# mobvoi/lstm_ctc

Measured on AMD Instinct MI355X. Metric: acoustic frames/sec (whole node), 5xBiLSTM-1024 CTC, higher is better.
Workload: dtype f32

## Files before the change

lstm_ctc_amd/csrc/lstm.hip:

```cpp
#include "common.h"
#include <stdlib.h>
#include <string.h>
#include <mutex>
#include <type_traits>

typedef float f32x4 __attribute__((ext_vector_type(4)));

static unsigned long long *g_lstm_dbg = nullptr;
typedef int x_i32x4 __attribute__((ext_vector_type(4)));
__device__ f32x4 x_buffer_load_b128(x_i32x4 rsrc, int voffset, int soffset, int aux) __asm("llvm.amdgcn.raw.buffer.load.v4f32");
__device__ void x_buffer_store_b128(f32x4 v, x_i32x4 rsrc, int voffset, int soffset, int aux) __asm("llvm.amdgcn.raw.buffer.store.v4f32");
typedef float x_f32x2v __attribute__((ext_vector_type(2)));
__device__ x_f32x2v x_buffer_load_b64(x_i32x4 rsrc, int voffset, int soffset, int aux) __asm("llvm.amdgcn.raw.buffer.load.v2f32");
__device__ float x_buffer_load_b32(x_i32x4 rsrc, int voffset, int soffset, int aux) __asm("llvm.amdgcn.raw.buffer.load.f32");
__device__ void x_buffer_store_b32(float v, x_i32x4 rsrc, int voffset, int soffset, int aux) __asm("llvm.amdgcn.raw.buffer.store.f32");
__device__ void x_buffer_store_b64(x_f32x2v v, x_i32x4 rsrc, int voffset, int soffset, int aux) __asm("llvm.amdgcn.raw.buffer.store.v2f32");
__device__ void x_buffer_store_b16(short v, x_i32x4 rsrc, int voffset, int soffset, int aux) __asm("llvm.amdgcn.raw.buffer.store.i16");

namespace {

constexpr int NTHREADS = 256;
constexpr int NWAVES = 4;

struct DirFwd {
// ... 1562 lines not shown
    for (int kb = 0; kb < NKB; ++kb) {
        const int k0 = uh * HALF + wave * (16 * NKB) + kb * 16 + 4 * lk;
#pragma unroll
        for (int c = 0; c < 8; ++c) {
            const int unit = ((c & 1) ? (1 - uh) : uh) * HALF + slot * 16 + li;
            const float *src = d.R + (size_t)k0 * G + (unit >> 3) * 32 + (c >> 1) * 8 + (unit & 7);
            wreg[kb][c].x = src[0]; wreg[kb][c].y = src[(size_t)G];
            wreg[kb][c].z = src[(size_t)2 * G]; wreg[kb][c].w = src[(size_t)3 * G];
        }
    }
    float *hxme = p.hx + (size_t)xcc * 2 * 2 * X_HXBUF;
    const x_i32x4 px_rs = x_rsrc(p.px, (unsigned)(X_PX_FLOATS * sizeof(float)));
    const int pxcell = ((slot * 16 + i) * 16 + ul) * 32;
    const x_i32x4 hx_rs = x_rsrc(hxme, (unsigned)(2 * 2 * X_HXBUF * sizeof(float)));
    const int hx_vo = (lk * 16 + li) * 16;
    const int hx_so = __builtin_amdgcn_readfirstlane(wave * NKB * 1024);
    const int hx_pub = (ul & 3) == 0 ? ((slot * 4 + (ul >> 2)) * 16 + i) * 16 : 0x7ffffff0;
    constexpr int X_NT = 2;
    auto publish_state = [&](int sg, int s, float h) {
        const int v = (int)((__float_as_uint(h) & ~1u) | p_gen_bit((unsigned)s + 1u));
        const f32x4 g = {__int_as_float(__builtin_amdgcn_mov_dpp(v, 0x00, 0xf, 0xf, true)),
                         __int_as_float(__builtin_amdgcn_mov_dpp(v, 0x55, 0xf, 0xf, true)),
                         __int_as_float(__builtin_amdgcn_mov_dpp(v, 0xaa, 0xf, 0xf, true)),
                         __int_as_float(__builtin_amdgcn_mov_dpp(v, 0xff, 0xf, 0xf, true))};
        x_buffer_store_b128(g, hx_rs, hx_pub, (sg * 2 + (s & 1)) * (X_HXBUF * 4), 0);
    };
    XGroup grp[2];
    grp[0].cprev = grp[1].cprev = 0.f;
    f32x4 a[NKB];
    bool failed = false;
    int step = 0;

    const x_i32x4 zx_rs = x_rsrc(d.zx, (unsigned)((size_t)T * B * G * sizeof(float)));
    const x_i32x4 cs_rs = x_rsrc(d.cs, (unsigned)((size_t)T * B * N * sizeof(float)));
    const x_i32x4 hs_rs = x_rsrc(d.hs, (unsigned)((size_t)T * B * N * sizeof(float)));
    int zvo[2], svo[2];
#pragma unroll
    for (int sg = 0; sg < 2; ++sg) { zvo[sg] = (brow[sg] * G + (int)zcol) * 4; svo[sg] = (brow[sg] * N + n) * 4; }
    auto load_zx = [&](int sg, int s) {
        const int zo = (int)((unsigned)(d.reverse ? (T - 1 - s) : s) * (unsigned)(B * G * 4));
#pragma unroll
        for (int g = 0; g < 4; ++g) grp[sg].z[g] = x_buffer_load_b32(zx_rs, zvo[sg] + 32 * g, zo, 0);
    };
    auto gates = [&](int sg, int s, const float (&zsum)[4]) {
        const int t = d.reverse ? (T - 1 - s) : s;
        const float cp = grp[sg].cprev;
        const float ia = lc_sigmoid(__builtin_fmaf(wi, cp, grp[sg].z[0] + zsum[0]));
        const float fa = lc_sigmoid(__builtin_fmaf(wf, cp, (grp[sg].z[2] + zsum[2]) + p.forget_bias));
        const float ja = lc_tanh(grp[sg].z[1] + zsum[1]);
        const float cn = __builtin_fmaf(fa, cp, ia * ja);
        const float oa = lc_sigmoid(__builtin_fmaf(wo, cn, grp[sg].z[3] + zsum[3]));
        const bool act = t < len[sg];
        const float h = act ? oa * lc_tanh(cn) : 0.f;
        grp[sg].cprev = act ? cn : 0.f;
        publish_state(sg, s, h);
        if (valid[sg]) {
            float *zrow = d.zx + ((size_t)t * B + brow[sg]) * G + zcol;
            const size_t so = ((size_t)t * B + brow[sg]) * N + n;
            zrow[0] = act ? ia : 0.f; zrow[8] = act ? ja : 0.f; zrow[16] = act ? fa : 0.f; zrow[24] = act ? oa : 0.f;
            d.cs[so] = grp[sg].cprev;
            d.hs[so] = h;
        }
    };
    auto request_state = [&](int sg, int s) {
        const int so = hx_so + (sg * 2 + ((s + 1) & 1)) * (X_HXBUF * 4);
#pragma unroll
        for (int kb = 0; kb < NKB; ++kb) a[kb] = x_buffer_load_b128(hx_rs, hx_vo, so + kb * 1024, X_NT);
    };
    auto state_stale = [&](int s, const f32x4 (&av)[NKB]) {
        unsigned stale = 0;
#pragma unroll
        for (int kb = 0; kb < NKB; ++kb) stale |= __float_as_uint(av[kb].x) ^ p_gen_bit((unsigned)s);
        return __builtin_amdgcn_ballot_w64((stale & 1u) != 0) != 0;
    };

    load_zx(0, 0);
    load_zx(1, 0);
    {
        const float zero[4] = {0.f, 0.f, 0.f, 0.f};
        gates(0, 0, zero);
        gates(1, 0, zero);
    }
    if (T > 1) { load_zx(0, 1); load_zx(1, 1); }
    __syncthreads();
    auto half = [&](auto XC, auto PC, int s) -> bool {
        constexpr int X = decltype(XC)::value, Y = X ^ 1;
        constexpr bool POST = decltype(PC)::value;
        const int k = 2 * s + X, sy = (k - 1) >> 1;
        step = s;
        float *partX = p_lds + (size_t)X * (NWAVES * 16 * X_LDP), *partY = p_lds + (size_t)Y * (NWAVES * 16 * X_LDP);
        if (X == 0) LC_XSTAMP(0); else LC_XSTAMP(8);
        {
            if (k == 2) request_state(X, s);
            if (state_stale(s, a)) {
                unsigned nspin = 0;
                for (;;) {
                    if (!p_keep_waiting(nspin, p.spin_limit, p.ctl)) { failed = true; break; }
                    asm volatile("" ::: "memory");
                    request_state(X, s);
                    if (!state_stale(s, a)) break;
                }
            }
        }
        if (X == 0) LC_XSTAMP(1); else LC_XSTAMP(9);
        f32x4 acc[8];
#pragma unroll
        for (int c = 0; c < 8; ++c) acc[c] = (f32x4){0.f, 0.f, 0.f, 0.f};
        asm volatile("s_nop 7" : "+v"(acc[0]), "+v"(acc[1]), "+v"(acc[2]), "+v"(acc[3]), "+v"(acc[4]), "+v"(acc[5]),
                                 "+v"(acc[6]), "+v"(acc[7]) : : "memory");
        float pl[4][NWAVES], pr[4][NWAVES], zrem[4], zsum[4] = {0.f, 0.f, 0.f, 0.f};
        f32x4 rv0 = {0.f, 0.f, 0.f, 0.f}, rv1 = rv0;
        float gx = 0.f, ge = 0.f, ia = 0.f, fa = 0.f, ja = 0.f, cn = 0.f, oa = 0.f, th = 0.f, hh = 0.f;
        bool act = false;
        const float tag_y = __uint_as_float((unsigned)sy);
        const int pxblk = (sy + 1) & 1;
        const int pxsend = (((xcc ^ 1) * 2 + Y) * 2 + pxblk) * X_PXBLK + pxcell, pxrecv = ((xcc * 2 + Y) * 2 + pxblk) * X_PXBLK + pxcell;
        const int ty = d.reverse ? (T - 1 - sy) : sy;
        const unsigned tyu = (unsigned)sy;
        auto late = [&]() {
            return __builtin_amdgcn_ballot_w64(((__float_as_uint(rv0.y) ^ tyu) | (__float_as_uint(rv0.w) ^ tyu) |
                                                (__float_as_uint(rv1.y) ^ tyu) | (__float_as_uint(rv1.w) ^ tyu)) != 0) != 0;
        };
        constexpr int C_RECV = NKB - 4 > 2 ? NKB - 4 : 2, C_SUM = C_RECV + 1, C_GATE = C_RECV + 2;
        static_assert(C_GATE < NKB, "five chunks at least");
        auto mic = [&](auto KC, int m) {
            constexpr int KB = decltype(KC)::value;
            XGroup &q = grp[Y];
            if constexpr (KB == 0 && POST) {
                const int g = m >> 3, w = (m >> 1) & 3;
                if (m & 1) pr[g][w] = partY[(size_t)(w * 16 + i) * X_LDP + g * 32 + 16 + ul];
                else pl[g][w] = partY[(size_t)(w * 16 + i) * X_LDP + g * 32 + ul];
            } else if constexpr (KB == 1 && POST) {
                if (m < 8) {
                    const int g = m >> 1;
                    if (m & 1) zrem[g] = (pr[g][0] + pr[g][1]) + (pr[g][2] + pr[g][3]);
                    else q.zloc[g] = (pl[g][0] + pl[g][1]) + (pl[g][2] + pl[g][3]);
                } else if (m == 8) {
                    x_buffer_store_b128((f32x4){zrem[0], tag_y, zrem[1], tag_y}, px_rs, pxsend, 0, X_SYS);
                } else if (m == 9) {
                    x_buffer_store_b128((f32x4){zrem[2], tag_y, zrem[3], tag_y}, px_rs, pxsend + 16, 0, X_SYS);
                }
            } else if constexpr (KB == C_RECV && POST) {
                if (m == 0) rv0 = x_buffer_load_b128(px_rs, pxrecv, 0, X_SYS);
                else if (m == 1) rv1 = x_buffer_load_b128(px_rs, pxrecv + 16, 0, X_SYS);
            } else if constexpr (KB == C_SUM && POST) {
                if (m == 0) {
                    if (late()) {
                        unsigned nspin = 0;
                        for (;;) {
                            if (!p_keep_waiting(nspin, p.spin_limit, p.ctl)) { failed = true; break; }
                            rv0 = x_buffer_load_b128(px_rs, pxrecv, 0, X_SYS);
                            rv1 = x_buffer_load_b128(px_rs, pxrecv + 16, 0, X_SYS);
                            if (!late()) break;
                        }
                    }
                } else if (m == 1) {
                    zsum[0] = q.zloc[0] + rv0.x; zsum[1] = q.zloc[1] + rv0.z;
                    zsum[2] = q.zloc[2] + rv1.x; zsum[3] = q.zloc[3] + rv1.z;
                }
            } else if constexpr (KB == C_GATE && POST) {
                const float cp = q.cprev;
                if (m == 0) gx = __builtin_fmaf(wi, cp, q.z[0] + zsum[0]);
                else if (m == 1) ge = __builtin_amdgcn_exp2f(-1.44269504088896341f * gx);
                else if (m == 2) ia = __builtin_amdgcn_rcpf(1.0f + ge);
                else if (m == 3) gx = __builtin_fmaf(wf, cp, (q.z[2] + zsum[2]) + p.forget_bias);
                else if (m == 4) ge = __builtin_amdgcn_exp2f(-1.44269504088896341f * gx);
                else if (m == 5) fa = __builtin_amdgcn_rcpf(1.0f + ge);
                else if (m == 6) { gx = q.z[1] + zsum[1]; ge = __builtin_amdgcn_exp2f(-2.88539008177792681f * fabsf(gx)); }
                else if (m == 7) ja = copysignf((1.0f - ge) * __builtin_amdgcn_rcpf(1.0f + ge), gx);
                else if (m == 8) { cn = __builtin_fmaf(fa, cp, ia * ja); gx = __builtin_fmaf(wo, cn, q.z[3] + zsum[3]); }
                else if (m == 9) ge = __builtin_amdgcn_exp2f(-1.44269504088896341f * gx);
                else if (m == 10) oa = __builtin_amdgcn_rcpf(1.0f + ge);
                else if (m == 11) ge = __builtin_amdgcn_exp2f(-2.88539008177792681f * fabsf(cn));
                else if (m == 12) th = copysignf((1.0f - ge) * __builtin_amdgcn_rcpf(1.0f + ge), cn);
                else if (m == 13) { act = ty < len[Y]; hh = act ? oa * th : 0.f; q.cprev = act ? cn : 0.f; }
                else if (m == 14) {
                    publish_state(Y, sy, hh);
                } else if (m == 16 || m == 18 || m == 20) {
                    if (valid[Y]) {
                        const int zo = (int)((unsigned)ty * (unsigned)(B * G * 4)), so = ty * B * N * 4;
                        if (m == 16) {
                            x_buffer_store_b32(act ? ia : 0.f, zx_rs, zvo[Y], zo, 0);
                            x_buffer_store_b32(act ? ja : 0.f, zx_rs, zvo[Y] + 32, zo, 0);
                        } else if (m == 18) {
                            x_buffer_store_b32(act ? fa : 0.f, zx_rs, zvo[Y] + 64, zo, 0);
                            x_buffer_store_b32(act ? oa : 0.f, zx_rs, zvo[Y] + 96, zo, 0);
                        } else {
                            x_buffer_store_b32(q.cprev, cs_rs, svo[Y], so, 0);
                            x_buffer_store_b32(hh, hs_rs, svo[Y], so, 0);
                        }
                    }
                } else if (m == 22) {
                    if (sy + 1 < T) load_zx(Y, sy + 1);
                }
            } else if constexpr (KB == C_GATE && !POST) {
                if (m == 0 && sy + 1 < T) load_zx(Y, sy + 1);
            }
        };
#define LC_XMFMA(ACC, A, W) asm volatile("v_mfma_f32_16x16x4_f32 %0, %1, %2, %0" : "+v"(ACC) : "v"(A), "a"(W))
#define LC_XCHUNK(KB)                                                                                              \
    _Pragma("unroll") for (int c = 0; c < 8; ++c) {                                                                \
        LC_XMFMA(acc[c], a[KB].x, wreg[KB][c].x); mic(std::integral_constant<int, KB>(), c);                       \
        __builtin_amdgcn_sched_barrier(0);                                                                         \
    }                                                                                                              \
    _Pragma("unroll") for (int c = 0; c < 8; ++c) {                                                                \
        LC_XMFMA(acc[c], a[KB].y, wreg[KB][c].y); mic(std::integral_constant<int, KB>(), 8 + c);                   \
        __builtin_amdgcn_sched_barrier(0);                                                                         \
    }                                                                                                              \
    _Pragma("unroll") for (int c = 0; c < 8; ++c) {                                                                \
        LC_XMFMA(acc[c], a[KB].z, wreg[KB][c].z); mic(std::integral_constant<int, KB>(), 16 + c);                  \
        __builtin_amdgcn_sched_barrier(0);                                                                         \
    }                                                                                                              \
    _Pragma("unroll") for (int c = 0; c < 8; ++c) {                                                                \
        LC_XMFMA(acc[c], a[KB].w, wreg[KB][c].w); mic(std::integral_constant<int, KB>(), 24 + c);                  \
        __builtin_amdgcn_sched_barrier(0);                                                                         \
    }
        LC_XCHUNK(0) LC_XCHUNK(1) LC_XCHUNK(2) LC_XCHUNK(3) LC_XCHUNK(4)
        if constexpr (NKB > 5) { LC_XCHUNK(5) }
        if constexpr (NKB > 6) { LC_XCHUNK(6) }
        if constexpr (NKB > 7) { LC_XCHUNK(7) }
#undef LC_XCHUNK
#undef LC_XMFMA
        asm volatile("s_nop 15\n\ts_nop 15\n\ts_nop 7" : "+v"(acc[0]), "+v"(acc[1]), "+v"(acc[2]), "+v"(acc[3]), "+v"(acc[4]),
                                                         "+v"(acc[5]), "+v"(acc[6]), "+v"(acc[7]) : : "memory");
        if (X == 0) LC_XSTAMP(2); else LC_XSTAMP(10);
#pragma unroll
        for (int c = 0; c < 8; ++c)
#pragma unroll
            for (int r = 0; r < 4; ++r) partX[(size_t)(wave * 16 + lk * 4 + r) * X_LDP + c * 16 + li] = acc[c][r];
        if (k + 1 < 2 * T) request_state(Y, (k + 1) >> 1);
        if (failed) s_fail = 1;
        __syncthreads();
        if (X == 0) LC_XSTAMP(3); else LC_XSTAMP(11);
        return s_fail == 0;
    };
    {
        const std::integral_constant<int, 0> g0;
        const std::integral_constant<int, 1> g1;
        const std::true_type post;
        bool ok = T > 1 && half(g0, std::false_type(), 1) && half(g1, post, 1);
        for (int s = 2; ok && s < T; ++s) ok = half(g0, post, s) && half(g1, post, s);
    }
    if (T > 1 && !s_fail) {
        const int Y = 1, sy = T - 1;
        const float *partY = p_lds + (size_t)Y * (NWAVES * 16 * X_LDP);
        const float tag_y = __uint_as_float((unsigned)sy);
        const int pxblk = (sy + 1) & 1;
        const int pxsend = (((xcc ^ 1) * 2 + Y) * 2 + pxblk) * X_PXBLK + pxcell, pxrecv = ((xcc * 2 + Y) * 2 + pxblk) * X_PXBLK + pxcell;
        float zrem[4], zsum[4];
#pragma unroll
        for (int g = 0; g < 4; ++g) {
            const float *q = partY + (size_t)i * X_LDP + g * 32 + ul;
            grp[Y].zloc[g] = (q[0] + q[(size_t)16 * X_LDP]) + (q[(size_t)32 * X_LDP] + q[(size_t)48 * X_LDP]);
            zrem[g] = (q[16] + q[(size_t)16 * X_LDP + 16]) + (q[(size_t)32 * X_LDP + 16] + q[(size_t)48 * X_LDP + 16]);
        }
        x_buffer_store_b128((f32x4){zrem[0], tag_y, zrem[1], tag_y}, px_rs, pxsend, 0, X_SYS);
        x_buffer_store_b128((f32x4){zrem[2], tag_y, zrem[3], tag_y}, px_rs, pxsend + 16, 0, X_SYS);
        unsigned nspin = 0;
        const unsigned ty = (unsigned)sy;
        f32x4 rv0, rv1;
        for (;;) {
            rv0 = x_buffer_load_b128(px_rs, pxrecv, 0, X_SYS);
            rv1 = x_buffer_load_b128(px_rs, pxrecv + 16, 0, X_SYS);
            if (__builtin_amdgcn_ballot_w64(((__float_as_uint(rv0.y) ^ ty) | (__float_as_uint(rv0.w) ^ ty) |
                                             (__float_as_uint(rv1.y) ^ ty) | (__float_as_uint(rv1.w) ^ ty)) != 0) == 0) break;
            if (!p_keep_waiting(nspin, p.spin_limit, p.ctl)) { failed = true; break; }
        }
        zsum[0] = grp[Y].zloc[0] + rv0.x; zsum[1] = grp[Y].zloc[1] + rv0.z;
        zsum[2] = grp[Y].zloc[2] + rv1.x; zsum[3] = grp[Y].zloc[3] + rv1.z;
        gates(Y, sy, zsum);
        if (__syncthreads_or(failed ? 1 : 0)) s_fail = 1;
    }
    if (s_fail && threadIdx.x == 0) p_report_failure(p.ctl);
}

constexpr int XB_LDP = 36;
typedef float x_f32x2 __attribute__((ext_vector_type(2)));
struct XBwdArgs {
    DirBwd d[2];
    const int *seq_len;
    int row_base[2];
    int T, B;
    unsigned spin_limit;
    PCtl *ctl;
    float *dzx;
    float *px;
    float *upg[2];
    unsigned long long *dbg;
};
constexpr int XB_DZBUF = 512 * 16 * 4;
constexpr size_t XB_DZX_FLOATS = (size_t)8 * 2 * 2 * XB_DZBUF;
constexpr int XB_PXBLK = 32 * 16 * 16 * 8;
constexpr size_t XB_PX_FLOATS = (size_t)8 * 2 * 2 * XB_PXBLK / 4;

struct XBGroup {
    float ia, ja, fa, oa, dh, cn, cp;
    float dc;
    float dloc;
};
template <int NKB>
__global__ __launch_bounds__(P_THREADS) void lstm_bwd_pair_kernel(XBwdArgs p)
{
    extern __shared__ __attribute__((aligned(16))) float p_lds[];
    __shared__ int s_slot, s_fail;
    const int xcc = p_xcc_id();
    if (xcc >= 8) return;
    if (threadIdx.x == 0) {
        s_fail = 0;
        s_slot = (int)__hip_atomic_fetch_add(&p.ctl->claim[xcc], 1u, __ATOMIC_RELAXED, __HIP_MEMORY_SCOPE_AGENT);
    }
    __syncthreads();
    const int slot = s_slot;
    constexpr int HALF = 64 * NKB, NSLOT = 4 * NKB, NB = 4 * NKB;
    if (slot >= NSLOT) return;
    const int dirx = xcc >> 2, rh = (xcc >> 1) & 1, uh = xcc & 1;
    const DirBwd &d = p.d[dirx];
    constexpr int N = 128 * NKB, G = 4 * N;
    const int B = p.B, T = p.T;
    const int lane = threadIdx.x & 63, wave = __builtin_amdgcn_readfirstlane(threadIdx.x >> 6);
    const int li = lane & 15, lk = lane >> 4;
    const int i = threadIdx.x >> 4, ul = threadIdx.x & 15;
    const int n = uh * HALF + slot * 16 + ul;
    const float wi = d.w_i ? d.w_i[n] : 0.f, wf = d.w_f ? d.w_f[n] : 0.f, wo = d.w_o ? d.w_o[n] : 0.f;
    const int cbase = (n >> 3) * 32 + (n & 7);
    int brow[2], len[2];
    bool valid[2];
#pragma unroll
    for (int sg = 0; sg < 2; ++sg) {
        const int b = p.row_base[dirx] + rh * 32 + sg * 16 + i;
        valid[sg] = b < B;
        brow[sg] = min(b, B - 1);
        len[sg] = valid[sg] ? p.seq_len[brow[sg]] : 0;
    }
    struct XW { float x, y, z, w; };
    XW wreg[NB][2];
#pragma unroll
    for (int kb = 0; kb < NB; ++kb) {
        const int ku = uh * HALF + wave * (16 * NKB) + kb * 4 + lk;
        const float *src0 = d.RT + (size_t)((ku >> 3) * 32 + (ku & 7)) * N;
#pragma unroll
        for (int c = 0; c < 2; ++c) {
            const int ou = (c ? (1 - uh) : uh) * HALF + slot * 16 + li;
            wreg[kb][c].x = src0[ou]; wreg[kb][c].y = src0[(size_t)8 * N + ou];
            wreg[kb][c].z = src0[(size_t)16 * N + ou]; wreg[kb][c].w = src0[(size_t)24 * N + ou];
        }
    }
    float *dzme = p.dzx + (size_t)xcc * 2 * 2 * XB_DZBUF;
    const x_i32x4 px_rs = x_rsrc(p.px, (unsigned)(XB_PX_FLOATS * sizeof(float)));
    const int pxcell = ((slot * 16 + i) * 16 + ul) * 8;
    const x_i32x4 dz_rs = x_rsrc(dzme, (unsigned)(2 * 2 * XB_DZBUF * sizeof(float)));
    const int dz_vo = (lk * 16 + li) * 16;
    const int dz_so = __builtin_amdgcn_readfirstlane(wave * NKB * 4096);
    const int dz_pub = ((slot * 16 + ul) * 16 + i) * 16;
    constexpr int X_NT = 2;
    XBGroup grp[2];
    grp[0].dc = grp[1].dc = 0.f;
    f32x4 a[2][16];
    float ug[2][7] = {{0.f, 0.f, 0.f, 0.f, 0.f, 0.f, 0.f}, {0.f, 0.f, 0.f, 0.f, 0.f, 0.f, 0.f}};
    auto uacc = [&](int sg, float gi, float gj, float gf, float go, float cp, float cn) {
        ug[sg][0] = __builtin_fmaf(gi, cp, ug[sg][0]); ug[sg][1] = __builtin_fmaf(gf, cp, ug[sg][1]);
        ug[sg][2] = __builtin_fmaf(go, cn, ug[sg][2]);
        ug[sg][3] += gi; ug[sg][4] += gj; ug[sg][5] += gf; ug[sg][6] += go;
    };
    bool failed = false;
    int step = 0;

    auto tof = [&](int s) { return d.reverse ? s : (T - 1 - s); };
    const x_i32x4 g_rs = x_rsrc(d.gates, (unsigned)((size_t)T * B * G * sizeof(float)));
    const x_i32x4 dh_rs = x_rsrc(d.dh, (unsigned)((size_t)T * B * N * sizeof(float)));
    const x_i32x4 cs_rs = x_rsrc(d.cs, (unsigned)((size_t)T * B * N * sizeof(float)));
    int gvo[2], svo[2];
#pragma unroll
    for (int sg = 0; sg < 2; ++sg) { gvo[sg] = (brow[sg] * G + cbase) * 4; svo[sg] = (brow[sg] * N + n) * 4; }
    auto load_gates = [&](int sg, int s) {
        const int go = (int)((unsigned)tof(s) * (unsigned)(B * G * 4));
        grp[sg].ia = x_buffer_load_b32(g_rs, gvo[sg], go, 0); grp[sg].ja = x_buffer_load_b32(g_rs, gvo[sg] + 32, go, 0);
        grp[sg].fa = x_buffer_load_b32(g_rs, gvo[sg] + 64, go, 0); grp[sg].oa = x_buffer_load_b32(g_rs, gvo[sg] + 96, go, 0);
    };
    auto load_rest = [&](int sg, int s) {
        const int t = tof(s);
        const int tprev = d.reverse ? t + 1 : t - 1;
        const bool has_prev = d.reverse ? (t + 1 < T) : (t > 0);
        grp[sg].dh = x_buffer_load_b32(dh_rs, svo[sg], t * B * N * 4, 0);
        grp[sg].cn = x_buffer_load_b32(cs_rs, svo[sg], t * B * N * 4, 0);
        const float cpv = x_buffer_load_b32(cs_rs, svo[sg], (has_prev ? tprev : t) * B * N * 4, 0);
        grp[sg].cp = has_prev ? cpv : 0.f;
    };
    auto load_operands = [&](int sg, int s) { load_gates(sg, s); load_rest(sg, s); };
    auto derivs = [&](int sg, int s, float drec) {
        const int t = tof(s);
        const XBGroup &q = grp[sg];
        const float dh = q.dh + drec;
        const float tc = lc_tanh(q.cn);
        const float do_pre = dh * tc * q.oa * (1.f - q.oa);
        const float dcn = __builtin_fmaf(do_pre, wo, __builtin_fmaf(dh * q.oa, __builtin_fmaf(-tc, tc, 1.f), q.dc));
        const float di_pre = dcn * q.ja * q.ia * (1.f - q.ia);
        const float dj_pre = dcn * q.ia * __builtin_fmaf(-q.ja, q.ja, 1.f);
        const float df_pre = dcn * q.cp * q.fa * (1.f - q.fa);
        const bool act = t < len[sg];
        const float odi = act ? di_pre : 0.f, odj = act ? dj_pre : 0.f, odf = act ? df_pre : 0.f, odo = act ? do_pre : 0.f;
        uacc(sg, odi, odj, odf, odo, q.cp, q.cn);
        grp[sg].dc = act ? __builtin_fmaf(df_pre, wf, __builtin_fmaf(di_pre, wi, dcn * q.fa)) : q.dc;
        x_buffer_store_b128(p_with_lsb_tag(odi, odj, odf, odo, p_gen_bit((unsigned)s + 1u)), dz_rs, dz_pub,
                            (sg * 2 + (s & 1)) * (XB_DZBUF * 4), 0);
        if (valid[sg]) {
            const int go = (int)((unsigned)t * (unsigned)(B * G * 4));
            x_buffer_store_b32(odi, g_rs, gvo[sg], go, 0); x_buffer_store_b32(odj, g_rs, gvo[sg] + 32, go, 0);
            x_buffer_store_b32(odf, g_rs, gvo[sg] + 64, go, 0); x_buffer_store_b32(odo, g_rs, gvo[sg] + 96, go, 0);
        }
    };
    auto request_dz = [&](auto SG, int s) {
        constexpr int sg = decltype(SG)::value;
        const int so = dz_so + (sg * 2 + ((s + 1) & 1)) * (XB_DZBUF * 4);
#pragma unroll
        for (int kb = 0; kb < 16; ++kb) a[sg][kb] = x_buffer_load_b128(dz_rs, dz_vo, so + kb * 1024, X_NT);
    };
    auto dz_stale = [&](auto SG, int s) {
        constexpr int sg = decltype(SG)::value;
        unsigned stale = 0;
        const unsigned gen = p_gen_bit((unsigned)s);
#pragma unroll
        for (int kb = 0; kb < 16; ++kb) stale |= __float_as_uint(a[sg][kb].x) ^ gen;
        return __builtin_amdgcn_ballot_w64((stale & 1u) != 0) != 0;
    };

    load_operands(0, 0);
    load_operands(1, 0);
    derivs(0, 0, 0.f);
    derivs(1, 0, 0.f);
    __syncthreads();
    auto half = [&](auto XC, auto PC, int s) -> bool {
        constexpr int X = decltype(XC)::value, Y = X ^ 1;
        constexpr bool POST = decltype(PC)::value;
        const int k = 2 * s + X, sy = (k - 1) >> 1;
        step = s;
        float *partX = p_lds + (size_t)X * (NWAVES * 16 * XB_LDP), *partY = p_lds + (size_t)Y * (NWAVES * 16 * XB_LDP);
        if (X == 0) LC_XSTAMP(0); else LC_XSTAMP(8);
        {
            if (k == 2) request_dz(XC, s);
            if (dz_stale(XC, s)) {
                unsigned nspin = 0;
                for (;;) {
                    if (!p_keep_waiting(nspin, p.spin_limit, p.ctl)) { failed = true; break; }
                    asm volatile("" ::: "memory");
                    request_dz(XC, s);
                    if (!dz_stale(XC, s)) break;
                }
            }
        }
        if (X == 0) LC_XSTAMP(1); else LC_XSTAMP(9);
        f32x4 acc[2][2];
#pragma unroll
        for (int c = 0; c < 2; ++c) acc[c][0] = acc[c][1] = (f32x4){0.f, 0.f, 0.f, 0.f};
        asm volatile("s_nop 7" : "+v"(acc[0][0]), "+v"(acc[0][1]), "+v"(acc[1][0]), "+v"(acc[1][1]) : : "memory");
        const int aso = dz_so + (X * 2 + ((s + 1) & 1)) * (XB_DZBUF * 4);
        const unsigned agen = p_gen_bit((unsigned)s);
        const int sn = (k + 1) >> 1, nso = dz_so + (Y * 2 + ((sn + 1) & 1)) * (XB_DZBUF * 4);
        float pl[NWAVES], pr[NWAVES];
        x_f32x2 rv = {0.f, 0.f};
        float dh = 0.f, tc = 0.f, ge = 0.f, psum = 0.f, do_pre = 0.f, dcn = 0.f, di_pre = 0.f, dj_pre = 0.f, df_pre = 0.f;
        float odi = 0.f, odj = 0.f, odf = 0.f, odo = 0.f;
        const float tag_y = __uint_as_float((unsigned)sy);
        const int pxblk = (sy + 1) & 1;
        const int pxsend = (((xcc ^ 1) * 2 + Y) * 2 + pxblk) * XB_PXBLK + pxcell, pxrecv = ((xcc * 2 + Y) * 2 + pxblk) * XB_PXBLK + pxcell;
        const int ty = tof(sy);
        const bool acty = ty < len[Y];
        constexpr int B_PUB = NB / 2, B_DER = B_PUB - 1, B_CHK = B_PUB - 2, B_RCV = B_PUB - 6 > 5 ? B_PUB - 6 : 5,
                      B_STO = B_PUB + 1, B_NXT = NB - 8;
        static_assert(B_RCV < B_CHK && B_STO < B_NXT + 8 && B_NXT >= B_PUB, "pair BPTT: block schedule");
        auto mic = [&](auto BC, int m) {
            constexpr int b = decltype(BC)::value;
            XBGroup &q = grp[Y];
            if constexpr (b >= 15 && b + 1 < NB) {
                if (m == 0) {
                    constexpr int kb = b + 1;
                    if (__builtin_amdgcn_ballot_w64(((__float_as_uint(a[X][kb & 15].x) ^ agen) & 1u) != 0) != 0) {
                        unsigned nspin = 0;
                        for (;;) {
                            if (!p_keep_waiting(nspin, p.spin_limit, p.ctl)) { failed = true; break; }
                            a[X][kb & 15] = x_buffer_load_b128(dz_rs, dz_vo, aso + kb * 1024, X_NT);
                            if (__builtin_amdgcn_ballot_w64(((__float_as_uint(a[X][kb & 15].x) ^ agen) & 1u) != 0) == 0) break;
                        }
                    }
                }
            }
            if constexpr (b >= B_NXT) {
                if (m == 1) a[Y][2 * (b - B_NXT)] = x_buffer_load_b128(dz_rs, dz_vo, nso + 2 * (b - B_NXT) * 1024, X_NT);
                else if (m == 2) a[Y][2 * (b - B_NXT) + 1] = x_buffer_load_b128(dz_rs, dz_vo, nso + (2 * (b - B_NXT) + 1) * 1024, X_NT);
            }
            if constexpr (POST) {
                if constexpr (b == 0) {
                    if (m < 4) pl[m] = partY[(size_t)(m * 16 + i) * XB_LDP + ul];
                } else if constexpr (b == 1) {
                    if (m < 4) pr[m] = partY[(size_t)(m * 16 + i) * XB_LDP + 16 + ul];
                } else if constexpr (b == 2) {
                    if (m == 0) load_gates(Y, sy);
                    else if (m == 2) load_rest(Y, sy);
                } else if constexpr (b == 3) {
                    if (m == 0) q.dloc = (pl[0] + pl[1]) + (pl[2] + pl[3]);
                    else if (m == 1) psum = (pr[0] + pr[1]) + (pr[2] + pr[3]);
                } else if constexpr (b == 4) {
                    if (m == 0) x_buffer_store_b64((x_f32x2){psum, tag_y}, px_rs, pxsend, 0, X_SYS);
                } else if constexpr (b == B_RCV) {
                    if (m == 0) rv = x_buffer_load_b64(px_rs, pxrecv, 0, X_SYS);
                } else if constexpr (b == B_CHK) {
                    if (m == 0) {
                        if (__builtin_amdgcn_ballot_w64(__float_as_uint(rv.y) != (unsigned)sy) != 0) {
                            unsigned nspin = 0;
                            for (;;) {
                                if (!p_keep_waiting(nspin, p.spin_limit, p.ctl)) { failed = true; break; }
                                rv = x_buffer_load_b64(px_rs, pxrecv, 0, X_SYS);
                                if (__builtin_amdgcn_ballot_w64(__float_as_uint(rv.y) != (unsigned)sy) == 0) break;
                            }
                        }
                    } else if (m == 1) dh = q.dh + (q.dloc + rv.x);
                    else if (m == 2) ge = __builtin_amdgcn_exp2f(-2.88539008177792681f * fabsf(q.cn));
                    else if (m == 3) tc = copysignf((1.0f - ge) * __builtin_amdgcn_rcpf(1.0f + ge), q.cn);
                } else if constexpr (b == B_DER) {
                    if (m == 1) do_pre = dh * tc * q.oa * (1.f - q.oa);
                    else if (m == 2) dcn = __builtin_fmaf(do_pre, wo, __builtin_fmaf(dh * q.oa, __builtin_fmaf(-tc, tc, 1.f), q.dc));
                    else if (m == 3) di_pre = dcn * q.ja * q.ia * (1.f - q.ia);
                    else if (m == 4) dj_pre = dcn * q.ia * __builtin_fmaf(-q.ja, q.ja, 1.f);
                    else if (m == 5) df_pre = dcn * q.cp * q.fa * (1.f - q.fa);
                    else if (m == 6) { odi = acty ? di_pre : 0.f; odj = acty ? dj_pre : 0.f; odf = acty ? df_pre : 0.f; odo = acty ? do_pre : 0.f; }
                    else if (m == 7) {
                        uacc(Y, odi, odj, odf, odo, q.cp, q.cn);
                        q.dc = acty ? __builtin_fmaf(df_pre, wf, __builtin_fmaf(di_pre, wi, dcn * q.fa)) : q.dc;
                    }
                } else if constexpr (b == B_PUB) {
                    if (m == 1)
                        x_buffer_store_b128(p_with_lsb_tag(odi, odj, odf, odo, p_gen_bit((unsigned)sy + 1u)), dz_rs, dz_pub,
                                            (Y * 2 + (sy & 1)) * (XB_DZBUF * 4), 0);
                } else if constexpr (b == B_STO) {
                    if (valid[Y]) {
                        const int go = (int)((unsigned)ty * (unsigned)(B * G * 4));
                        if (m == 1) { x_buffer_store_b32(odi, g_rs, gvo[Y], go, 0); x_buffer_store_b32(odj, g_rs, gvo[Y] + 32, go, 0); }
                        else if (m == 2) { x_buffer_store_b32(odf, g_rs, gvo[Y] + 64, go, 0); x_buffer_store_b32(odo, g_rs, gvo[Y] + 96, go, 0); }
                    }
                }
            }
            if constexpr (b + 16 < NB) {
                if (m == 7) a[X][b & 15] = x_buffer_load_b128(dz_rs, dz_vo, aso + (b + 16) * 1024, X_NT);
            }
        };
#define LC_XMFMA(ACC, A, W) asm volatile("v_mfma_f32_16x16x4_f32 %0, %1, %2, %0" : "+v"(ACC) : "v"(A), "a"(W))
#define LC_XM(KB, M, ACC, A, W)                                                                                    \
    LC_XMFMA(ACC, A, W); mic(std::integral_constant<int, KB>(), M); __builtin_amdgcn_sched_barrier(0);
#define LC_XB(KB)                                                                                                  \
    LC_XM(KB, 0, acc[0][0], a[X][(KB) & 15].x, wreg[KB][0].x) LC_XM(KB, 1, acc[1][0], a[X][(KB) & 15].x, wreg[KB][1].x) \
    LC_XM(KB, 2, acc[0][1], a[X][(KB) & 15].y, wreg[KB][0].y) LC_XM(KB, 3, acc[1][1], a[X][(KB) & 15].y, wreg[KB][1].y) \
    LC_XM(KB, 4, acc[0][0], a[X][(KB) & 15].z, wreg[KB][0].z) LC_XM(KB, 5, acc[1][0], a[X][(KB) & 15].z, wreg[KB][1].z) \
    LC_XM(KB, 6, acc[0][1], a[X][(KB) & 15].w, wreg[KB][0].w) LC_XM(KB, 7, acc[1][1], a[X][(KB) & 15].w, wreg[KB][1].w)
        LC_XB(0) LC_XB(1) LC_XB(2) LC_XB(3) LC_XB(4) LC_XB(5) LC_XB(6) LC_XB(7)
        LC_XB(8) LC_XB(9) LC_XB(10) LC_XB(11) LC_XB(12) LC_XB(13) LC_XB(14) LC_XB(15)
        LC_XB(16) LC_XB(17) LC_XB(18) LC_XB(19)
        if constexpr (NKB > 5) { LC_XB(20) LC_XB(21) LC_XB(22) LC_XB(23) }
        if constexpr (NKB > 6) { LC_XB(24) LC_XB(25) LC_XB(26) LC_XB(27) }
        if constexpr (NKB > 7) { LC_XB(28) LC_XB(29) LC_XB(30) LC_XB(31) }
#undef LC_XB
#undef LC_XM
#undef LC_XMFMA
        asm volatile("s_nop 15\n\ts_nop 15\n\ts_nop 7" : "+v"(acc[0][0]), "+v"(acc[0][1]), "+v"(acc[1][0]), "+v"(acc[1][1]) : : "memory");
        if (X == 0) LC_XSTAMP(2); else LC_XSTAMP(10);
#pragma unroll
        for (int c = 0; c < 2; ++c)
#pragma unroll
            for (int r = 0; r < 4; ++r)
                partX[(size_t)(wave * 16 + lk * 4 + r) * XB_LDP + c * 16 + li] = acc[c][0][r] + acc[c][1][r];
        if (failed) s_fail = 1;
        __syncthreads();
        if (X == 0) LC_XSTAMP(3); else LC_XSTAMP(11);
        return s_fail == 0;
    };
    {
        const std::integral_constant<int, 0> g0;
        const std::integral_constant<int, 1> g1;
        const std::true_type post;
        bool ok = T > 1 && half(g0, std::false_type(), 1) && half(g1, post, 1);
        for (int s = 2; ok && s < T; ++s) ok = half(g0, post, s) && half(g1, post, s);
    }
    if (T > 1 && !s_fail) {
        const int Y = 1, sy = T - 1;
        const float *q = p_lds + (size_t)Y * (NWAVES * 16 * XB_LDP) + (size_t)i * XB_LDP + ul;
        const float tag_y = __uint_as_float((unsigned)sy);
        const int pxblk = (sy + 1) & 1;
        const int pxsend = (((xcc ^ 1) * 2 + Y) * 2 + pxblk) * XB_PXBLK + pxcell, pxrecv = ((xcc * 2 + Y) * 2 + pxblk) * XB_PXBLK + pxcell;
        grp[Y].dloc = (q[0] + q[(size_t)16 * XB_LDP]) + (q[(size_t)32 * XB_LDP] + q[(size_t)48 * XB_LDP]);
        const float drem = (q[16] + q[(size_t)16 * XB_LDP + 16]) + (q[(size_t)32 * XB_LDP + 16] + q[(size_t)48 * XB_LDP + 16]);
        x_buffer_store_b64((x_f32x2){drem, tag_y}, px_rs, pxsend, 0, X_SYS);
        unsigned nspin = 0;
        x_f32x2 rv;
        for (;;) {
            rv = x_buffer_load_b64(px_rs, pxrecv, 0, X_SYS);
            if (__builtin_amdgcn_ballot_w64(__float_as_uint(rv.y) != (unsigned)sy) == 0) break;
            if (!p_keep_waiting(nspin, p.spin_limit, p.ctl)) { failed = true; break; }
        }
        load_operands(Y, sy);
        derivs(Y, sy, grp[Y].dloc + rv.x);
        if (__syncthreads_or(failed ? 1 : 0)) s_fail = 1;
    }
    if (p.upg[dirx]) {
#pragma unroll
        for (int sg = 0; sg < 2; ++sg) {
            float *o = p.upg[dirx] + (size_t)(rh * 32 + sg * 16 + i) * 7 * N + n;
#pragma unroll
            for (int k = 0; k < 7; ++k) o[(size_t)k * N] = ug[sg][k];
        }
    }
    if (s_fail && threadIdx.x == 0) p_report_failure(p.ctl);
}

#include "lstm_pair_x3.inc"

inline size_t al256(size_t x) { return (x + 255) & ~(size_t)255; }
inline bool persist_device_ok()
{
    static std::mutex mu;
    static int state[16] = {0};
    int dev = 0;
    if (hipGetDevice(&dev) != hipSuccess || dev < 0 || dev >= 16) { (void)hipGetLastError(); return false; }
    std::lock_guard<std::mutex> lock(mu);
    if (state[dev] == 0) {
        hipDeviceProp_t prop;
        int xccs = 0;
        const bool ok = hipGetDeviceProperties(&prop, dev) == hipSuccess &&
                        hipDeviceGetAttribute(&xccs, hipDeviceAttributeNumberOfXccs, dev) == hipSuccess &&
                        strncmp(prop.gcnArchName, "gfx950", 6) == 0 && prop.multiProcessorCount == 256 && xccs == 8;
        if (!ok) (void)hipGetLastError();
        state[dev] = ok ? 1 : -1;
    }
    return state[dev] == 1;
}
inline unsigned persist_spin_limit()
{
    const long v = lc_option(LC_OPT_LSTM_SPIN_LIMIT, P_SPIN_LIMIT);
    return v < 0 ? 0u : (unsigned)v;
}
thread_local int g_last_sched = 0;
inline bool persist_geom(int T, int B, int N, int ndir, bool bwd, PGeom &g, size_t &lds_bytes)
{
    if (lc_option(LC_OPT_LSTM_PERSISTENT, 1) == 0 || N > P_MAXN || N % 16 != 0 || T < 4 || !persist_device_ok()) return false;
    g.T = T; g.B = B; g.N = N; g.ndir = ndir;
    g.gpd = 8 / ndir;
    g.rpg = lc_cdiv(B, g.gpd);
    if (g.rpg > 16) return false;
    g.upw = (lc_cdiv(N, 32) + 3) & ~3;
    g.UP = g.upw;
    g.nwg = lc_cdiv(N, g.upw);
    (void)bwd;
    lds_bytes = 84 * 1024;
    return true;
}
inline bool persist_geom_bf16(int T, int B, int N, int ndir, PGeom &g, size_t &lds_bytes)
{
    if (lc_option(LC_OPT_LSTM_PERSISTENT, 1) == 0 || N > 1024 || N % 32 != 0 || T < 4 || !persist_device_ok()) return false;
    g.T = T; g.B = B; g.N = N; g.ndir = ndir;
    g.gpd = 8 / ndir;
    g.rpg = lc_cdiv(B, g.gpd);
    if (g.rpg > 16) return false;
    g.upw = (lc_cdiv(N, 32) + 3) & ~3;
    g.UP = g.upw;
    g.nwg = lc_cdiv(N, g.upw);
    lds_bytes = 84 * 1024;
    return true;
}
inline bool pair_width(int N) { return N == 640 || N == 768 || N == 896 || N == 1024; }
inline bool pair_x3_width(int N) { return N == 768 || N == 1024; }
inline bool persist_x3_width(int N) { return N >= 64 && N <= 512 && N % 64 == 0; }
inline bool pair_geom(int T, int B, int N, int ndir)
{
    return lc_option(LC_OPT_LSTM_PERSISTENT, 1) != 0 && pair_width(N) && (ndir == 1 || ndir == 2) && B >= 1 && T >= 4 &&
           (unsigned long long)T * B * 4 * N * sizeof(float) <= 0xffffffffull && persist_device_ok();
}
inline int pair_rows_per_launch(int ndir) { return ndir == 2 ? 64 : 128; }
inline size_t pair_fwd_ws_bytes() { return P_CTL_BYTES + (X_HX_FLOATS + X_PX_FLOATS) * sizeof(float); }
inline size_t pair_bwd_ws_bytes() { return P_CTL_BYTES + (XB_DZX_FLOATS + XB_PX_FLOATS) * sizeof(float); }
inline size_t pair_bwd_x3_ws_bytes() { return P_CTL_BYTES + (X3B_DZX_FLOATS + XB_PX_FLOATS) * sizeof(float); }
inline size_t persist_ws_bytes(int N, bool bwd)
{
    if (N > 1024 || N % 16 != 0) return 0;
    return P_CTL_BYTES + (size_t)8 * 2 * (bwd ? 4 * N : 2 * N) * 16 * sizeof(float);
}
inline size_t persist_bwd_x3_ws_bytes(int N) { return P_CTL_BYTES + (size_t)8 * 2 * x3p_bwd_buf_bytes(N); }
inline size_t upg_part_bytes(int N) { return al256((size_t)2 * UPG_SPLITS * 7 * N * sizeof(float)); }

inline int bpad(int B) { return B <= 16 ? 16 : (B <= 64 ? ((B + 31) & ~31) : ((B + 63) & ~63)); }

inline bool persist_clear(void *workspace, size_t ws_bytes, hipStream_t s, int fill = 0)
{
    return hipMemsetAsync(workspace, 0, LC_LSTM_STATUS_OFFSET, s) == hipSuccess &&
           hipMemsetAsync((char *)workspace + P_CTL_BYTES, fill, ws_bytes - P_CTL_BYTES, s) == hipSuccess;
}

template <class K, class A>
inline bool persist_launch(K kernel, size_t lds, hipStream_t s, const A &args)
{
    if (hipFuncSetAttribute((const void *)kernel, hipFuncAttributeMaxDynamicSharedMemorySize, (int)lds) != hipSuccess)
        return false;
    hipLaunchKernelGGL(kernel, dim3(P_GRID), dim3(P_THREADS), lds, s, args);
    return true;
}

}

extern "C" void lc_debug_set_lstm_stamps(unsigned long long *buf) { g_lstm_dbg = buf; }
extern "C" int lc_debug_last_lstm_schedule(void) { return g_last_sched; }

extern "C" size_t lc_lstm_fwd_workspace_bytes(int B, int N, int ndir)
{
    size_t need = P_CTL_BYTES + (size_t)ndir * (al256((size_t)2 * N * bpad(B) * sizeof(float)) +
                                                al256((size_t)N * 4 * N * sizeof(float)));
    if (al256(persist_ws_bytes(N, false)) > need) need = al256(persist_ws_bytes(N, false));
    if (pair_width(N) && al256(pair_fwd_ws_bytes()) > need) need = al256(pair_fwd_ws_bytes());
    return need;
}
static size_t lstm_bwd_main_bytes(int B, int N, int ndir)
{
    size_t need = P_CTL_BYTES + (size_t)ndir * (al256((size_t)2 * 4 * N * bpad(B) * sizeof(float)) +
                                                al256((size_t)B * N * sizeof(float)) +
                                                al256((size_t)N * 4 * N * sizeof(float)));
    if (al256(persist_ws_bytes(N, true)) > need) need = al256(persist_ws_bytes(N, true));
    if (pair_width(N) && al256(pair_bwd_ws_bytes()) > need) need = al256(pair_bwd_ws_bytes());
    if (pair_x3_width(N) && al256(pair_bwd_x3_ws_bytes()) > need) need = al256(pair_bwd_x3_ws_bytes());
    if (persist_x3_width(N) && al256(persist_bwd_x3_ws_bytes(N)) > need) need = al256(persist_bwd_x3_ws_bytes(N));
    return need;
}
extern "C" size_t lc_lstm_bwd_workspace_bytes(int B, int N, int ndir)
{
    return lstm_bwd_main_bytes(B, N, ndir) + upg_part_bytes(N);
}

struct DirStreams {
    hipStream_t s_hi, s_lo;
    int prio_hi;
    hipEvent_t fork, join;
};
static DirStreams *dir_streams(hipStream_t caller, hipStream_t *second)
{
    static DirStreams pool[16];
    static int state[16] = {0};
    static std::mutex mu;
    int dev = 0;
    if (hipGetDevice(&dev) != hipSuccess || dev < 0 || dev >= 16) return nullptr;
    DirStreams &d = pool[dev];
    {
        std::lock_guard<std::mutex> lock(mu);
        if (state[dev] == 0) {
            int lo = 0, hi = 0;
            const bool ok = hipDeviceGetStreamPriorityRange(&lo, &hi) == hipSuccess && lo != hi &&
                            hipStreamCreateWithPriority(&d.s_hi, hipStreamNonBlocking, hi) == hipSuccess &&
                            hipStreamCreateWithPriority(&d.s_lo, hipStreamNonBlocking, lo) == hipSuccess &&
                            hipEventCreateWithFlags(&d.fork, hipEventDisableTiming) == hipSuccess &&
                            hipEventCreateWithFlags(&d.join, hipEventDisableTiming) == hipSuccess;
            d.prio_hi = hi;
            state[dev] = ok ? 1 : -1;
            if (!ok) (void)hipGetLastError();
        }
        if (state[dev] != 1) return nullptr;
    }
    int prio = 0;
    if (hipStreamGetPriority(caller, &prio) != hipSuccess) { (void)hipGetLastError(); prio = 0; }
    *second = (prio == d.prio_hi) ? d.s_lo : d.s_hi;
    return &d;
}

static void pack_operand(bool bf, const float *W, int K, int C, void *dst, hipStream_t s)
{
    if (bf) hipLaunchKernelGGL(pack_k32_bf16_kernel, dim3(1024), dim3(256), 0, s, W, K, C, (unsigned short *)dst);
    else hipLaunchKernelGGL(pack_k16_kernel, dim3(1024), dim3(256), 0, s, W, K, C, (float *)dst);
}

template <bool BF>
static void launch_fwd_step(int mt, dim3 grid, hipStream_t s, const FwdArgs &a)
{
    dim3 block(NTHREADS);
    switch (mt) {
    case 1: hipLaunchKernelGGL((lstm_fwd_step_kernel<1, BF>), grid, block, 0, s, a); break;
    case 2: hipLaunchKernelGGL((lstm_fwd_step_kernel<2, BF>), grid, block, 0, s, a); break;
    case 3: hipLaunchKernelGGL((lstm_fwd_step_kernel<3, BF>), grid, block, 0, s, a); break;
    default: hipLaunchKernelGGL((lstm_fwd_step_kernel<4, BF>), grid, block, 0, s, a); break;
    }
}

static int lstm_fwd_impl(bool bf, bool x3, const char *who, const lc_lstm_fwd_dir_t *dirs, int ndir, const int *seq_len, int T,
                         int B, int N, float forget_bias, void *workspace, size_t workspace_bytes, lc_stream_t stream)
{
    LC_CHECK_ARG(dirs && seq_len && workspace, "%s: null pointer", who);
    LC_CHECK_ARG(ndir == 1 || ndir == 2, "%s: ndir must be 1 or 2", who);
    LC_CHECK_ARG(T > 0 && B > 0 && N > 0 && N % (bf ? 32 : 16) == 0, "%s: need T,B > 0 and num_neurons %% %d == 0 (N=%d)",
                 who, bf ? 32 : 16, N);
    if (workspace_bytes < lc_lstm_fwd_workspace_bytes(B, N, ndir)) {
        lc_set_error("%s: workspace too small", who);
        return LC_EWORKSPACE;
    }
    for (int i = 0; i < ndir; ++i)
        LC_CHECK_ARG(dirs[i].zx && dirs[i].R && dirs[i].cs && dirs[i].hs, "%s: null pointer in dirs[%d]", who, i);
    hipStream_t s = (hipStream_t)stream;
    if (!bf && pair_geom(T, B, N, ndir)) {
        XFwdArgs xa;
        for (int i = 0; i < 2; ++i) {
            const lc_lstm_fwd_dir_t &di = dirs[ndir == 2 ? i : 0];
            xa.d[i].zx = di.zx; xa.d[i].R = di.R;
            xa.d[i].w_f = di.w_f; xa.d[i].w_i = di.w_i; xa.d[i].w_o = di.w_o;
            xa.d[i].cs = di.cs; xa.d[i].hs = di.hs; xa.d[i].hT = nullptr; xa.d[i].reverse = di.reverse;
        }
        xa.seq_len = seq_len; xa.T = T; xa.B = B; xa.forget_bias = forget_bias;
        xa.spin_limit = persist_spin_limit();
        xa.ctl = (PCtl *)workspace;
        xa.hx = (float *)((char *)workspace + P_CTL_BYTES);
        xa.px = xa.hx + X_HX_FLOATS;
        xa.dbg = g_lstm_dbg;
        for (int r0 = 0; r0 < B; r0 += pair_rows_per_launch(ndir)) {
            xa.row_base[0] = r0;
            xa.row_base[1] = ndir == 2 ? r0 : r0 + 64;
            if (!persist_clear(workspace, pair_fwd_ws_bytes(), s)) {
                lc_set_error("%s: memset failed", who);
                return LC_ELAUNCH;
            }
            const bool use_x3 = x3 && pair_x3_width(N);
            const bool launched = use_x3 ? (N == 1024 ? persist_launch(lstm_fwd_pair_x3_kernel<8>, x3_fwd_lds_bytes(8), s, xa)
                                                      : persist_launch(lstm_fwd_pair_x3_kernel<6>, x3_fwd_lds_bytes(6), s, xa))
                                : N == 1024 ? persist_launch(lstm_fwd_pair_kernel<8>, (size_t)84 * 1024, s, xa)
                                : N == 896 ? persist_launch(lstm_fwd_pair_kernel<7>, (size_t)84 * 1024, s, xa)
                                : N == 768 ? persist_launch(lstm_fwd_pair_kernel<6>, (size_t)84 * 1024, s, xa)
                                           : persist_launch(lstm_fwd_pair_kernel<5>, (size_t)84 * 1024, s, xa);
            if (!launched) {
                lc_set_error("%s: hipFuncSetAttribute(MaxDynamicSharedMemorySize) failed for the XCD-pair kernel", who);
                (void)hipGetLastError();
                return LC_ELAUNCH;
            }
            PVerifyArgs va;
            va.ctl = xa.ctl; va.nused = 8; va.nwg = N / 32; va.nout = ndir;
            va.out[0] = dirs[0].hs; va.out[1] = dirs[ndir - 1].hs; va.count = va.count16 = (size_t)T * B * N;
            va.out16[0] = va.out16[1] = nullptr;
            hipLaunchKernelGGL(persist_verify_kernel, dim3(256), dim3(256), 0, s, va);
            LC_CHECK_LAUNCH("lstm_fwd_pair");
        }
        g_last_sched = x3 && pair_x3_width(N) ? 6 : 5;
        return LC_OK;
    }
    PFwdArgs pa;
    size_t lds = 0;
    const bool persist = bf ? persist_geom_bf16(T, B, N, ndir, pa.g, lds) : persist_geom(T, B, N, ndir, false, pa.g, lds);
    if (persist) {
        for (int i = 0; i < ndir; ++i) {
            pa.d[i].zx = dirs[i].zx; pa.d[i].R = dirs[i].R;
            pa.d[i].w_f = dirs[i].w_f; pa.d[i].w_i = dirs[i].w_i; pa.d[i].w_o = dirs[i].w_o;
            pa.d[i].cs = dirs[i].cs; pa.d[i].hs = dirs[i].hs; pa.d[i].hT = nullptr; pa.d[i].reverse = dirs[i].reverse;
            pa.d[i].hs16 = bf ? dirs[i].hs_bf16 : nullptr;
        }
        if (ndir == 1) pa.d[1] = pa.d[0];
        pa.seq_len = seq_len; pa.forget_bias = forget_bias;
        pa.spin_limit = persist_spin_limit();
        pa.ctl = (PCtl *)workspace;
        pa.hT = (float *)((char *)workspace + P_CTL_BYTES);
        pa.dbg = bf ? nullptr : g_lstm_dbg;
        if (!persist_clear(workspace, persist_ws_bytes(N, false), s, bf ? 0xff : 0)) {
            lc_set_error("%s: memset failed", who);
            return LC_ELAUNCH;
        }
        bool ok = false;
        const bool px3 = !bf && x3 && persist_x3_width(N);
        if (px3) {
#define LC_PFX(NB) case NB: ok = persist_launch(lstm_fwd_persist_x3_kernel<NB>, lds, s, pa); break;
            switch (N / 32) { LC_PFX(2) LC_PFX(4) LC_PFX(6) LC_PFX(8) LC_PFX(10) LC_PFX(12) LC_PFX(14) LC_PFX(16) }
#undef LC_PFX
        } else if (!bf) {
            const int per = lc_cdiv(N / 16, NWAVES);
#define LC_PFWD(PER)                                                                                                   \
    case PER:                                                                                                          \
        ok = (N % 64) ? persist_launch(lstm_fwd_persist_kernel<PER, true>, lds, s, pa)                                 \
                      : persist_launch(lstm_fwd_persist_kernel<PER, false>, lds, s, pa);                               \
        break;
            switch (per) { LC_PFWD(1) LC_PFWD(2) LC_PFWD(3) LC_PFWD(4) LC_PFWD(5) LC_PFWD(6) LC_PFWD(7) LC_PFWD(8) }
#undef LC_PFWD
        } else {
            const int perb = lc_cdiv(N / 32, NWAVES);
#define LC_PFB(PERB, PPT)                                                                                              \
    case PERB:                                                                                                         \
        ok = (N % 128) ? persist_launch(lstm_fwd_persist_bf16_kernel<PERB, PPT, true>, lds, s, pa)                     \
                       : persist_launch(lstm_fwd_persist_bf16_kernel<PERB, PPT, false>, lds, s, pa);                   \
        break;
            bool shonly = N == 1024;
            for (int i = 0; i < ndir; ++i) shonly = shonly && dirs[i].shadow_only && dirs[i].hs_bf16;
            if (shonly) ok = persist_launch(lstm_fwd_persist_bf16_kernel<8, 2, false, true>, lds, s, pa);
            else
            switch (perb) { LC_PFB(1, 1) LC_PFB(2, 1) LC_PFB(3, 1) LC_PFB(4, 1) LC_PFB(5, 2) LC_PFB(6, 2) LC_PFB(7, 2) LC_PFB(8, 2) }
#undef LC_PFB
        }
        if (!ok) {
            lc_set_error("%s: hipFuncSetAttribute(MaxDynamicSharedMemorySize) failed for the persistent kernel", who);
            (void)hipGetLastError();
            return LC_ELAUNCH;
        }
        PVerifyArgs va;
        va.ctl = pa.ctl; va.nused = ndir * pa.g.gpd; va.nwg = pa.g.nwg; va.nout = ndir;
        va.out[0] = dirs[0].hs; va.out[1] = dirs[ndir - 1].hs; va.count = va.count16 = (size_t)T * B * N;
        va.out16[0] = bf ? (unsigned short *)dirs[0].hs_bf16 : nullptr;
        va.out16[1] = bf ? (unsigned short *)dirs[ndir - 1].hs_bf16 : nullptr;
        hipLaunchKernelGGL(persist_verify_kernel, dim3(256), dim3(256), 0, s, va);
        LC_CHECK_LAUNCH(bf ? "lstm_fwd_persist_bf16" : "lstm_fwd_persist");
        g_last_sched = (bf ? 2 : px3 ? 7 : 1) | ((int)bf << 16);
        return LC_OK;
    }
    FwdArgs a;
    a.seq_len = seq_len; a.T = T; a.B = B; a.N = N; a.Bpad = bpad(B); a.forget_bias = forget_bias;
    a.dbg = g_lstm_dbg;
    char *w = (char *)workspace + P_CTL_BYTES;
    for (int i = 0; i < ndir; ++i) {
        a.d[i].zx = dirs[i].zx;
        a.d[i].w_f = dirs[i].w_f; a.d[i].w_i = dirs[i].w_i; a.d[i].w_o = dirs[i].w_o;
        a.d[i].cs = dirs[i].cs; a.d[i].hs = dirs[i].hs; a.d[i].reverse = dirs[i].reverse;
// ... 307 lines not shown
```

Measured before the change: 190,000.

## Defer MFMA partial-sum LDS writes into next half-step and drop trailing barrier

In the persistent backward pair kernel, each half-step no longer drains its MFMA accumulators with long s_nop padding, writes partials to LDS, and ends on __syncthreads. Accumulators are now kept per half (accs[X]) and written to LDS inside the next half's MFMA stream. The failure flag moves into a per-wave LDS array that is read back after a single s_barrier placed mid-stream. The first MFMAs of the next half now zero-initialise their accumulators directly and are tied to the previous accumulators, which keeps those registers live. The goal is to remove one block-wide barrier and the drain latency per half-step and overlap them with MFMA work, at the cost of more accumulator register pressure and a more fragile hand-written sync/hazard ordering.

```diff
diff --git a/lstm_ctc_amd/csrc/lstm.hip b/lstm_ctc_amd/csrc/lstm.hip
--- a/lstm_ctc_amd/csrc/lstm.hip
+++ b/lstm_ctc_amd/csrc/lstm.hip
@@ -1888,11 +1888,12 @@
 __global__ __launch_bounds__(P_THREADS) void lstm_bwd_pair_kernel(XBwdArgs p)
 {
     extern __shared__ __attribute__((aligned(16))) float p_lds[];
-    __shared__ int s_slot, s_fail;
+    __shared__ int s_slot;
+    __shared__ __attribute__((aligned(16))) int s_flag[2][NWAVES];
     const int xcc = p_xcc_id();
     if (xcc >= 8) return;
+    if (threadIdx.x < 2 * NWAVES) (&s_flag[0][0])[threadIdx.x] = 0;
     if (threadIdx.x == 0) {
-        s_fail = 0;
         s_slot = (int)__hip_atomic_fetch_add(&p.ctl->claim[xcc], 1u, __ATOMIC_RELAXED, __HIP_MEMORY_SCOPE_AGENT);
     }
     __syncthreads();
@@ -1942,6 +1943,7 @@
     XBGroup grp[2];
     grp[0].dc = grp[1].dc = 0.f;
     f32x4 a[2][16];
+    f32x4 accs[2][2][2];
     float ug[2][7] = {{0.f, 0.f, 0.f, 0.f, 0.f, 0.f, 0.f}, {0.f, 0.f, 0.f, 0.f, 0.f, 0.f, 0.f}};
     auto uacc = [&](int sg, float gi, float gj, float gf, float go, float cp, float cn) {
         ug[sg][0] = __builtin_fmaf(gi, cp, ug[sg][0]); ug[sg][1] = __builtin_fmaf(gf, cp, ug[sg][1]);
@@ -2020,7 +2022,7 @@
         constexpr bool POST = decltype(PC)::value;
         const int k = 2 * s + X, sy = (k - 1) >> 1;
         step = s;
-        float *partX = p_lds + (size_t)X * (NWAVES * 16 * XB_LDP), *partY = p_lds + (size_t)Y * (NWAVES * 16 * XB_LDP);
+        float *partY = p_lds + (size_t)Y * (NWAVES * 16 * XB_LDP);
         if (X == 0) LC_XSTAMP(0); else LC_XSTAMP(8);
         {
             if (k == 2) request_dz(XC, s);
@@ -2035,10 +2037,8 @@
             }
         }
         if (X == 0) LC_XSTAMP(1); else LC_XSTAMP(9);
-        f32x4 acc[2][2];
-#pragma unroll
-        for (int c = 0; c < 2; ++c) acc[c][0] = acc[c][1] = (f32x4){0.f, 0.f, 0.f, 0.f};
-        asm volatile("s_nop 7" : "+v"(acc[0][0]), "+v"(acc[0][1]), "+v"(acc[1][0]), "+v"(acc[1][1]) : : "memory");
+        f32x4 (&acc)[2][2] = accs[X];
+        x_i32x4 gone = {0, 0, 0, 0};
         const int aso = dz_so + (X * 2 + ((s + 1) & 1)) * (XB_DZBUF * 4);
         const unsigned agen = p_gen_bit((unsigned)s);
         const int sn = (k + 1) >> 1, nso = dz_so + (Y * 2 + ((sn + 1) & 1)) * (XB_DZBUF * 4);
@@ -2076,9 +2076,28 @@
             }
             if constexpr (POST) {
                 if constexpr (b == 0) {
-                    if (m < 4) pl[m] = partY[(size_t)(m * 16 + i) * XB_LDP + ul];
+                    if (m >= 4) {
+                        const int c = (m - 4) >> 1;
+#pragma unroll
+                        for (int e = 0; e < 2; ++e) {
+                            const int r = ((m - 4) & 1) * 2 + e;
+                            partY[(size_t)(wave * 16 + lk * 4 + r) * XB_LDP + c * 16 + li] = accs[Y][c][0][r] + accs[Y][c][1][r];
+                        }
+                    }
                 } else if constexpr (b == 1) {
-                    if (m < 4) pr[m] = partY[(size_t)(m * 16 + i) * XB_LDP + 16 + ul];
+                    if (m == 0) {
+                        s_flag[k & 1][wave] = failed ? 1 : 0;
+                        asm volatile("s_waitcnt lgkmcnt(0)" ::: "memory");
+                        __builtin_amdgcn_s_barrier();
+                        asm volatile("" ::: "memory");
+                        gone = *reinterpret_cast<const x_i32x4 *>(&s_flag[k & 1][0]);
+                    } else if (m < 3) {
+#pragma unroll
+                        for (int w = 2 * (m - 1); w < 2 * m; ++w) pl[w] = partY[(size_t)(w * 16 + i) * XB_LDP + ul];
+                    } else if (m < 5) {
+#pragma unroll
+                        for (int w = 2 * (m - 3); w < 2 * (m - 2); ++w) pr[w] = partY[(size_t)(w * 16 + i) * XB_LDP + 16 + ul];
+                    }
                 } else if constexpr (b == 2) {
                     if (m == 0) load_gates(Y, sy);
                     else if (m == 2) load_rest(Y, sy);
@@ -2130,8 +2149,19 @@
             }
         };
 #define LC_XMFMA(ACC, A, W) asm volatile("v_mfma_f32_16x16x4_f32 %0, %1, %2, %0" : "+v"(ACC) : "v"(A), "a"(W))
+#define LC_XM0 "v_mfma_f32_16x16x4_f32 %"
+#define LC_XMFMA0_TEXT LC_XM0 "0, %4, %6, 0\n\t" LC_XM0 "1, %4, %7, 0\n\t" LC_XM0 "2, %5, %8, 0\n\t" LC_XM0 "3, %5, %9, 0"
+#define LC_XMFMA0_OUT "=&v"(acc[0][0]), "=&v"(acc[1][0]), "=&v"(acc[0][1]), "=&v"(acc[1][1])
+#define LC_XMFMA0_IN "v"(a[X][0].x), "v"(a[X][0].y), "a"(wreg[0][0].x), "a"(wreg[0][1].x), "a"(wreg[0][0].y), "a"(wreg[0][1].y)
+#define LC_XMFMA0()                                                                                                \
+    if constexpr (POST)                                                                                            \
+        asm volatile(LC_XMFMA0_TEXT : LC_XMFMA0_OUT : LC_XMFMA0_IN, "v"(accs[Y][0][0]), "v"(accs[Y][0][1]),        \
+                     "v"(accs[Y][1][0]), "v"(accs[Y][1][1]));                                                      \
+    else asm volatile(LC_XMFMA0_TEXT : LC_XMFMA0_OUT : LC_XMFMA0_IN)
 #define LC_XM(KB, M, ACC, A, W)                                                                                    \
-    LC_XMFMA(ACC, A, W); mic(std::integral_constant<int, KB>(), M); __builtin_amdgcn_sched_barrier(0);
+    if constexpr ((KB) == 0 && (M) < 4) { if constexpr ((M) == 0) { LC_XMFMA0(); } }      \
+    else { LC_XMFMA(ACC, A, W); mic(std::integral_constant<int, KB>(), M); }                                       \
+    __builtin_amdgcn_sched_barrier(0);
 #define LC_XB(KB)                                                                                                  \
     LC_XM(KB, 0, acc[0][0], a[X][(KB) & 15].x, wreg[KB][0].x) LC_XM(KB, 1, acc[1][0], a[X][(KB) & 15].x, wreg[KB][1].x) \
     LC_XM(KB, 2, acc[0][1], a[X][(KB) & 15].y, wreg[KB][0].y) LC_XM(KB, 3, acc[1][1], a[X][(KB) & 15].y, wreg[KB][1].y) \
@@ -2145,18 +2175,14 @@
         if constexpr (NKB > 7) { LC_XB(28) LC_XB(29) LC_XB(30) LC_XB(31) }
 #undef LC_XB
 #undef LC_XM
+#undef LC_XMFMA0
+#undef LC_XMFMA0_IN
+#undef LC_XMFMA0_OUT
+#undef LC_XMFMA0_TEXT
+#undef LC_XM0
 #undef LC_XMFMA
-        asm volatile("s_nop 15\n\ts_nop 15\n\ts_nop 7" : "+v"(acc[0][0]), "+v"(acc[0][1]), "+v"(acc[1][0]), "+v"(acc[1][1]) : : "memory");
-        if (X == 0) LC_XSTAMP(2); else LC_XSTAMP(10);
-#pragma unroll
-        for (int c = 0; c < 2; ++c)
-#pragma unroll
-            for (int r = 0; r < 4; ++r)
-                partX[(size_t)(wave * 16 + lk * 4 + r) * XB_LDP + c * 16 + li] = acc[c][0][r] + acc[c][1][r];
-        if (failed) s_fail = 1;
-        __syncthreads();
-        if (X == 0) LC_XSTAMP(3); else LC_XSTAMP(11);
-        return s_fail == 0;
+        if (X == 0) { LC_XSTAMP(2); LC_XSTAMP(3); } else { LC_XSTAMP(10); LC_XSTAMP(11); }
+        return (gone.x | gone.y | gone.z | gone.w) == 0;
     };
     {
         const std::integral_constant<int, 0> g0;
@@ -2165,9 +2191,18 @@
         bool ok = T > 1 && half(g0, std::false_type(), 1) && half(g1, post, 1);
         for (int s = 2; ok && s < T; ++s) ok = half(g0, post, s) && half(g1, post, s);
     }
-    if (T > 1 && !s_fail) {
+    bool lost = __syncthreads_or(failed ? 1 : 0) != 0;
+    if (T > 1 && !lost) {
         const int Y = 1, sy = T - 1;
-        const float *q = p_lds + (size_t)Y * (NWAVES * 16 * XB_LDP) + (size_t)i * XB_LDP + ul;
+        float *partY = p_lds + (size_t)Y * (NWAVES * 16 * XB_LDP);
+        asm volatile("s_nop 15\n\ts_nop 15\n\ts_nop 7" : "+v"(accs[Y][0][0]), "+v"(accs[Y][0][1]), "+v"(accs[Y][1][0]), "+v"(accs[Y][1][1]) : : "memory");
+#pragma unroll
+        for (int c = 0; c < 2; ++c)
+#pragma unroll
+            for (int r = 0; r < 4; ++r)
+                partY[(size_t)(wave * 16 + lk * 4 + r) * XB_LDP + c * 16 + li] = accs[Y][c][0][r] + accs[Y][c][1][r];
+        __syncthreads();
+        const float *q = partY + (size_t)i * XB_LDP + ul;
         const float tag_y = __uint_as_float((unsigned)sy);
         const int pxblk = (sy + 1) & 1;
         const int pxsend = (((xcc ^ 1) * 2 + Y) * 2 + pxblk) * XB_PXBLK + pxcell, pxrecv = ((xcc * 2 + Y) * 2 + pxblk) * XB_PXBLK + pxcell;
@@ -2183,7 +2218,7 @@
         }
         load_operands(Y, sy);
         derivs(Y, sy, grp[Y].dloc + rv.x);
-        if (__syncthreads_or(failed ? 1 : 0)) s_fail = 1;
+        lost = __syncthreads_or(failed ? 1 : 0) != 0;
     }
     if (p.upg[dirx]) {
 #pragma unroll
@@ -2193,7 +2228,7 @@
             for (int k = 0; k < 7; ++k) o[(size_t)k * N] = ug[sg][k];
         }
     }
-    if (s_fail && threadIdx.x == 0) p_report_failure(p.ctl);
+    if (lost && threadIdx.x == 0) p_report_failure(p.ctl);
 }
 
 #include "lstm_pair_x3.inc"
```

Result: no change. 190,800 (median of 6 runs) (+0.4%).
